# JuliaNeuralGraphics/GaussianSplatting.jl

Measured on AMD Instinct MI355X. Metric: fwd+bwd Mpixels/s @1920x1080, 1M Gaussians SH=3, higher is better.
Workload: dtype f32

## Files before the change

gaussiansplatting.jl_amd/csrc/gsr_api.cpp:

```cpp
#include "../../include/gsr.h"

#include <dlfcn.h>
#include <math.h>
#include <sched.h>
#include <time.h>
#include <hip/hip_runtime.h>

#include <algorithm>
#include <atomic>
#include <chrono>
#include <cstdarg>
#include <cstdio>
#include <cstdlib>
#include <cstring>
#include <new>
#include <vector>

#include "gsr_kernels.h"
#include "adam_math.h"

namespace {

thread_local char g_err[512] = "";

// ... 863 lines not shown

static int buffer_lookup(const gsr_handle* h, int which, const void** dev_ptr, size_t* bytes) {
    const size_t n = (size_t)h->last_n, P = (size_t)h->cfg.width * h->cfg.height, T = (size_t)h->n_tiles;
    const size_t D = (size_t)h->last_D;
    const DevBuf* b = nullptr;
    size_t sz = 0;
    switch (which) {
        case GSR_BUF_RADII:
            *dev_ptr = h->fwd_valid && n ? h->radii_cur : nullptr;
            *bytes = *dev_ptr ? n * 4 : 0;
            return GSR_OK;
        case GSR_BUF_GRAD_MEANS2D:
            *dev_ptr = h->bwd_valid && n ? h->vmean2d_cur : nullptr;
            *bytes = *dev_ptr ? n * 8 : 0;
            return GSR_OK;
        case GSR_BUF_N_CONTRIB: b = &h->n_contrib; sz = P * 4; break;
        case GSR_BUF_FINAL_T: b = &h->final_T; sz = P * 4; break;
        case GSR_BUF_TILE_RANGES: b = &h->ranges; sz = 2 * T * 4; break;
        case GSR_BUF_VALUES_SORTED: b = &h->values_sorted; sz = h->fwd_only ? 0 : D * 4; break;
        case GSR_BUF_GEOM: b = &h->geo; sz = n * 64; break;
        case GSR_BUF_NORMALS: b = &h->gnormal; sz = h->cfg.mode > 5 ? n * 16 : 0; break;
        case GSR_BUF_GRAD_ROWS: b = &h->rows; sz = (size_t)h->last_slots * 16 * GSR_ROW_F4(h->cfg.mode); break;
        case GSR_BUF_INSTANCE_AUX: b = &h->s2; sz = h->fwd_only ? 0 : D * 16; break;
        default: return fail(GSR_E_INVALID_ARG, "unknown buffer id %d", which);
    }
    if (sz > b->cap) sz = 0;
    *dev_ptr = sz ? b->p : nullptr;
    *bytes = sz;
    return GSR_OK;
}

int gsr_buffer(const gsr_handle* h, int which, const void** dev_ptr, size_t* bytes) {
    if (!h || !dev_ptr || !bytes) return fail(GSR_E_INVALID_ARG, "null argument");
    return buffer_lookup(h, which, dev_ptr, bytes);
}

int gsr_copy_buffer(const gsr_handle* h, int which, void* dst, size_t bytes, void* stream) {
    if (!h || (!dst && bytes)) return fail(GSR_E_INVALID_ARG, "null argument");
    const void* src = nullptr;
    size_t have = 0;
    int rc = buffer_lookup(h, which, &src, &have);
    if (rc) return rc;
    if (bytes > have) return fail(GSR_E_STATE, "buffer %d holds %zu bytes, %zu requested (not produced yet?)", which, have, bytes);
    if (bytes) HIPCHK(hipMemcpyAsync(dst, src, bytes, hipMemcpyDeviceToDevice, (hipStream_t)stream));
    return GSR_OK;
}

int gsr_ssim_forward(int W, int H, int CH, int B, const float* img, const float* ref, float C1, float C2, int train,
                     float* ssim_map, float* dm_dmu1, float* dm_dsigma1_sq, float* dm_dsigma12, void* stream) {
    if (W <= 0 || H <= 0 || CH <= 0 || B <= 0) return fail(GSR_E_INVALID_ARG, "bad SSIM shape");
    if (!img || !ref || !ssim_map) return fail(GSR_E_INVALID_ARG, "null SSIM array");
    if (train && (!dm_dmu1 || !dm_dsigma1_sq || !dm_dsigma12)) return fail(GSR_E_INVALID_ARG, "train needs the 3 partial maps");
    if ((size_t)CH * B > 65535) return fail(GSR_E_INVALID_ARG, "CH*B too large");
    (g_ssim_exact.load(std::memory_order_relaxed) ? gsr_launch_ssim_fwd_exact : gsr_launch_ssim_fwd_fast)((hipStream_t)stream, W, H, CH, B, img, ref, C1, C2, train,
                                                                          ssim_map, dm_dmu1, dm_dsigma1_sq, dm_dsigma12);
    HIPCHK(hipGetLastError());
    return GSR_OK;
}

int gsr_ssim_backward(int W, int H, int CH, int B, const float* img, const float* ref, const float* dL_dmap,
                      const float* dm_dmu1, const float* dm_dsigma1_sq, const float* dm_dsigma12, float* dL_dimg,
                      void* stream) {
    if (W <= 0 || H <= 0 || CH <= 0 || B <= 0) return fail(GSR_E_INVALID_ARG, "bad SSIM shape");
    if (!img || !ref || !dL_dmap || !dm_dmu1 || !dm_dsigma1_sq || !dm_dsigma12 || !dL_dimg)
        return fail(GSR_E_INVALID_ARG, "null SSIM array");
    if ((size_t)CH * B > 65535) return fail(GSR_E_INVALID_ARG, "CH*B too large");
    (g_ssim_exact.load(std::memory_order_relaxed) ? gsr_launch_ssim_bwd_exact : gsr_launch_ssim_bwd_fast)((hipStream_t)stream, W, H, CH, B, img, ref, dL_dmap, dm_dmu1,
                                                                          dm_dsigma1_sq, dm_dsigma12, dL_dimg);
    HIPCHK(hipGetLastError());
    return GSR_OK;
}

int gsr_loss_l1_ssim(gsr_handle* h, const float* image, const float* target, float lambda_dssim, float* loss_out,
                     float* vpixels, void* stream) {
    if (!h || !image || !target || !loss_out || !vpixels) return fail(GSR_E_INVALID_ARG, "null argument");
    hipStream_t s = (hipStream_t)stream;
    const int W = h->cfg.width, H = h->cfg.height, C = h->cfg.mode;
    const size_t P = (size_t)W * H;
    int rc;
    if ((rc = h->d0.ensure(3 * P * 4)) || (rc = h->d1.ensure(3 * P * 4)) || (rc = h->d2.ensure(3 * P * 4)) ||
        (rc = h->partial.ensure((size_t)h->n_tiles * 3 * 2 * 4)))
        return rc;
    const float C1 = 0.01f * 0.01f, C2 = 0.03f * 0.03f;
    const int exact = ssim_exact_of(h);
    StageScope sc9(h->prof, ST_LOSS_FWD, s);
    (exact ? gsr_launch_loss_fwd_exact : gsr_launch_loss_fwd_fast)(s, W, H, C, image, target, C1, C2, h->d0.as<float>(),
                                                                          h->d1.as<float>(), h->d2.as<float>(), h->partial.as<float>());
    sc9.close();
    StageScope sc10(h->prof, ST_LOSS_BWD, s);
    (exact ? gsr_launch_loss_bwd_exact : gsr_launch_loss_bwd_fast)(s, W, H, C, image, target, lambda_dssim, h->d0.as<float>(),
                                                                          h->d1.as<float>(), h->d2.as<float>(), h->partial.as<float>(),
                                                                          loss_out, vpixels);
    sc10.close();
    HIPCHK(hipGetLastError());
    h->loss_vpixels = vpixels;
    h->loss_generation = h->generation;
    return GSR_OK;
}

int gsr_update_stats(gsr_handle* h, int32_t* max_radii, float* accum_grad_means2d, float* denom, void* stream) {
    if (!h || !max_radii || !accum_grad_means2d || !denom) return fail(GSR_E_INVALID_ARG, "null argument");
    if (!h->fwd_valid || !h->bwd_valid) return fail(GSR_E_STATE, "gsr_update_stats needs a completed forward/backward pair");
    gsr_launch_update_stats((hipStream_t)stream, h->last_n, h->radii_cur, h->vmean2d_cur,
                            h->cfg.width, h->cfg.height, max_radii, accum_grad_means2d, denom);
    HIPCHK(hipGetLastError());
    return GSR_OK;
}

int gsr_profile_enable(gsr_handle* h, int on) {
    if (!h) return fail(GSR_E_INVALID_ARG, "null handle");
    h->prof.on = (on & 1) != 0;
    h->prof.ranges = (on & 2) != 0;
    if (!h->prof.on) h->prof.clear();
    return GSR_OK;
}

int gsr_profile_stages(gsr_handle* h, uint32_t stage_mask) {
    if (!h) return fail(GSR_E_INVALID_ARG, "null handle");
    h->prof.mask = stage_mask;
    return GSR_OK;
}

int gsr_profile_stage_count(void) { return ST_COUNT; }
const char* gsr_profile_stage_name(int stage) { return stage >= 0 && stage < ST_COUNT ? kStageNames[stage] : ""; }

int gsr_profile_read(gsr_handle* h, double* ms_sum, int* launches, int reset) {
    if (!h || !ms_sum || !launches) return fail(GSR_E_INVALID_ARG, "null argument");
    for (int i = 0; i < ST_COUNT; i++) { ms_sum[i] = 0.0; launches[i] = 0; }
    for (auto& r : h->prof.recs) {
        float ms = 0.0f;
        HIPCHK(hipEventSynchronize(r.b));
        HIPCHK(hipEventElapsedTime(&ms, r.a, r.b));
        ms_sum[r.stage] += ms;
        if (!r.extra) launches[r.stage] += 1;
    }
    if (reset) h->prof.clear();
    return GSR_OK;
// ... 476 lines not shown
```

gaussiansplatting.jl_amd/csrc/gsr_kernels.h:

```cpp
#pragma once
#include <hip/hip_runtime.h>
#include <stdint.h>

#define GSR_TILE 16
#define GSR_BATCH 256
#define GSR_SORT_LDS_CAP 8192

struct GsrCam {
    float R[9];
    float t[3];
    float focal[2];
    float principal[2];
    float center[3];
    int width, height;
    int grid_x, grid_y;
    float near_plane, far_plane;
    int radius_clip;
    float blur_eps;
    int exact_cull;
    const float* R_dev;
    const float* t_dev;
};

struct GsrGeoRec { float4 q0, q1, q2, q3; };
// ... 92 lines not shown
                              const float* final_T, GsrInst inst,
                              uint32_t split_len ,
                              bool color_only ,
                              bool accurate );
void gsr_launch_composite_bwd_listed(hipStream_t s, int channels, GsrCam cam, const uint32_t* tile_start,
                                     GsrTierLists tiers, GsrStream stream, const float* background,
                                     const float* vpixels, const uint32_t* n_contrib, const float* final_T, GsrInst inst,
                                     float* long_state );

#define GSR_ADAM_MAX_GROUPS 8
void gsr_launch_prologue_fwd(hipStream_t s, int n, int k_rest, int scale_dims, const float* sh_color,
                             const float* sh_remainder, const float* opacities, const float* scales, float* shs,
                             float* opacities_act, float* scales_act);
void gsr_launch_prologue_bwd(hipStream_t s, int n, int k_rest, int scale_dims, const float* opacities_act,
                             const float* scales_act, const float* vshs, const float* vopacities_act,
                             const float* vscales_act, float* v_sh_color, float* v_sh_remainder, float* v_opacities,
                             float* v_scales);
void gsr_launch_adam(hipStream_t s, int n_groups, float* const* theta, const float* const* grad, float* const* mu,
                     float* const* nu, const long long* count, const float* lr_t, float beta1, float beta2, float eps);

void gsr_launch_trainer_tail(hipStream_t s, int n, int k_rest, int scale_dims, const float* const* grads,
                             float* const* theta, float* const* mu, float* const* nu, const float* lr_t, float beta1,
                             float beta2, float eps, float* shs, float* opac_act, float* scales_act);
size_t gsr_findall_scratch_bytes(long long n);
void gsr_launch_findall(hipStream_t s, long long n, const uint8_t* mask, uint32_t* indices, uint32_t* count_dev,
                        uint32_t* scratch);
void gsr_launch_gather_rows(hipStream_t s, int n_groups, const void* const* src, void* const* dst, const int* row_words,
                            const uint32_t* idx, long long count);
void gsr_launch_triad(hipStream_t s, size_t n4, float* a, const float* b, const float* c, float q);

#define GSR_COMPOSE_MAX_GROUPS 24
void gsr_launch_grad_mean(hipStream_t s, long long n, const float* accum, const float* denom, float* out);
void gsr_launch_densify_mask(hipStream_t s, int kind, long long n, long long n_grad, const float* grad, const float* scales,
                             int scale_dims, const float* opacities, const int32_t* max_radii, float thr, float gamma,
                             float min_opacity, int max_screen_size, uint8_t* mask);
void gsr_launch_compose_rows(hipStream_t s, int n_groups, const void* const* src, void* const* dst, const int* row_words,
                             const int* new_zero, const uint32_t* keep_idx, long long n_keep, const uint32_t* sel_idx,
                             long long n_sel, int reps);
void gsr_launch_split_transform(hipStream_t s, long long n_new, int scale_dims, float* points, const float* rots,
                                float* scales, uint32_t seed);
void gsr_launch_reset_opacity(hipStream_t s, long long n, float* opacities);
void gsr_launch_morton_codes(hipStream_t s, long long n, const float* points, const float lo[3], const float inv_extent[3],
                             unsigned long long* codes);
void gsr_launch_nonfinite_scan(hipStream_t s, int n_groups, const float* const* src, const int* row_words, long long n_rows,
                               uint32_t* counts, uint32_t* first_bad);
void gsr_launch_ply_rows(hipStream_t s, bool pack, long long n, int kr, float* points, float* dc, float* rest, float* opac,
                         float* scales, float* rots, float* rows);

#define GSR_SSIM_DECL(SUF)                                                                                              \
    void gsr_launch_ssim_fwd_##SUF(hipStream_t s, int W, int H, int CH, int B, const float* img, const float* ref, float C1, \
                                   float C2, int train, float* ssim_map, float* d0, float* d1, float* d2);             \
    void gsr_launch_ssim_bwd_##SUF(hipStream_t s, int W, int H, int CH, int B, const float* img, const float* ref,      \
                                   const float* dL_dmap, const float* d0, const float* d1, const float* d2, float* dL_dimg); \
              \
    void gsr_launch_loss_fwd_##SUF(hipStream_t s, int W, int H, int C, const float* image, const float* target, float C1, \
                                   float C2, float* d0, float* d1, float* d2, float* partial);                         \
    void gsr_launch_loss_bwd_##SUF(hipStream_t s, int W, int H, int C, const float* image, const float* target, float lambda, \
                                   const float* d0, const float* d1, const float* d2, const float* partial, float* loss_out, \
                                   float* vpixels);
GSR_SSIM_DECL(exact)
GSR_SSIM_DECL(fast)
#undef GSR_SSIM_DECL

namespace gsr {
struct AdamHyper;
struct BilateralTv { float weight, nx, ny, nz, n12, rx, ry, rz; };
}
int gsr_bilateral_chunks(int W, int H, int gx, int gy);
size_t gsr_bilateral_partial_bytes(int W, int H, int gx, int gy, int gz);
void gsr_launch_bilateral_fwd(hipStream_t s, int W, int H, int C, const float* image, const float* grid, int gx, int gy,
                              int gz, float* out);
void gsr_launch_bilateral_bwd(hipStream_t s, int W, int H, int C, const float* image, const float* grid, int gx, int gy,
                              int gz, const float* vout, float* vimage, float* vgrid, float* partial);
void gsr_launch_bilateral_tv(hipStream_t s, int n, int gx, int gy, int gz, const float* grids, const gsr::BilateralTv& tv,
                             float* loss_out, float* grad_out, float* partial);
void gsr_launch_bilateral_adam_tail(hipStream_t s, int n, int gx, int gy, int gz, float* grids, float* mu, float* nu,
                                    const float* vgrid, int view, const gsr::BilateralTv& tv, const gsr::AdamHyper& h,
                                    float* tv_loss_out, float* partial);
```

gaussiansplatting.jl_amd/csrc/ssim.hip:

```cpp
#include "gsr_kernels.h"

#ifndef SSIM_EXACT
#define SSIM_EXACT 1
#endif
#if SSIM_EXACT
#define SSIM_NAME(x) x##_exact
#else
#define SSIM_NAME(x) x##_fast
#endif

namespace {

constexpr int HALO = 5;
constexpr int SH_DIM = GSR_TILE + 2 * HALO;
constexpr int IN_STRIDE = 48, HC_STRIDE = 16;

__constant__ float GAUSS[11] = {0.001028380123898387f, 0.0075987582094967365f, 0.036000773310661316f,
                                0.10936068743467331f,  0.21300552785396576f,   0.26601171493530273f,
                                0.21300552785396576f,  0.10936068743467331f,   0.036000773310661316f,
                                0.0075987582094967365f, 0.001028380123898387f};

struct PlanarSrc {
    const float* img;
    const float* ref;
    int W, H;
    __device__ __forceinline__ float x(int gx, int gy, int plane) const {
        return img[(size_t)gx + (size_t)W * gy + (size_t)W * H * plane];
    }
    __device__ __forceinline__ float y(int gx, int gy, int plane) const {
        return ref[(size_t)gx + (size_t)W * gy + (size_t)W * H * plane];
    }
};
struct RasterSrc {
    const float* image;
    const float* target;
    int W, H, C;
    __device__ __forceinline__ float x(int gx, int gy, int plane) const {
        return image[(size_t)C * ((size_t)gx + (size_t)W * gy) + plane];
    }
    __device__ __forceinline__ float y(int gx, int gy, int plane) const {
        return target[(size_t)gx + (size_t)W * gy + (size_t)W * H * plane];
    }
};

__device__ __forceinline__ bool ssim_tile_of_block(int W, int H, int& tx0, int& ty0) {
    const int gx = (W + GSR_TILE - 1) / GSR_TILE, gy = (H + GSR_TILE - 1) / GSR_TILE;
    const int n = gx * gy, per = (n + 7) / 8;
    const int t = (int)(blockIdx.x & 7) * per + (int)(blockIdx.x >> 3);
    if ((int)(blockIdx.x >> 3) >= per || t >= n) return false;
    tx0 = (t % gx) * GSR_TILE;
    ty0 = (t / gx) * GSR_TILE;
    return true;
}

__device__ __forceinline__ float block_sum(float v, float* red ) {
#pragma unroll
    for (int off = 32; off > 0; off >>= 1) v += __shfl_xor(v, off);
    if ((threadIdx.x & 63) == 0) red[threadIdx.x >> 6] = v;
    __syncthreads();
    float r = red[0] + red[1] + red[2] + red[3];
    __syncthreads();
    return r;
}

template <class Src, bool LOSS, int NCH>
__global__ __launch_bounds__(256) void ssim_fwd_kernel(Src src, int W, int H, float C1, float C2, int train,
                                                       float* __restrict__ ssim_map, float* __restrict__ d0,
                                                       float* __restrict__ d1, float* __restrict__ d2,
                                                       float* __restrict__ partial) {
    __shared__ float sx[SH_DIM][IN_STRIDE], sy[SH_DIM][IN_STRIDE];
    __shared__ float hc[5][SH_DIM][HC_STRIDE];
    __shared__ float red[4];
    const int tid = threadIdx.x, tx = tid & 15, ty = tid >> 4;
    int x0, y0;
    const bool live = ssim_tile_of_block(W, H, x0, y0);
    float l1 = 0.0f, sv = 0.0f;
    if (!live) {
        if (LOSS && tid == 0) { partial[2 * ((size_t)blockIdx.x + (size_t)gridDim.x * blockIdx.z)] = 0.0f; partial[2 * ((size_t)blockIdx.x + (size_t)gridDim.x * blockIdx.z) + 1] = 0.0f; }
        return;
    }
  for (int ch = 0; ch < NCH; ch++) {
    const int plane = blockIdx.z * NCH + ch;
    if (ch > 0) __syncthreads();
    for (int f = tid; f < SH_DIM * SH_DIM; f += 256) {
        const int ly = f / SH_DIM, lx = f - ly * SH_DIM;
        const int gx = x0 + lx - HALO, gy = y0 + ly - HALO;
        const bool in = gx >= 0 && gx < W && gy >= 0 && gy < H;
        sx[ly][lx] = in ? src.x(gx, gy, plane) : 0.0f;
        sy[ly][lx] = in ? src.y(gx, gy, plane) : 0.0f;
    }
    __syncthreads();
    for (int r = ty; r < SH_DIM; r += GSR_TILE) {
        const int cx = tx + HALO;
        float s0 = 0, s1 = 0, s2 = 0, s3 = 0, s4 = 0;
#pragma unroll
        for (int d = 1; d <= HALO; d++) {
            const float w = GAUSS[HALO - d];
            const float Xl = sx[r][cx - d], Yl = sy[r][cx - d], Xr = sx[r][cx + d], Yr = sy[r][cx + d];
            s0 += (Xl + Xr) * w;
            s1 += (Xl * Xl + Xr * Xr) * w;
            s2 += (Yl + Yr) * w;
            s3 += (Yl * Yl + Yr * Yr) * w;
            s4 += (Xl * Yl + Xr * Yr) * w;
        }
        const float Xc = sx[r][cx], Yc = sy[r][cx], wc = GAUSS[HALO];
        s0 += Xc * wc; s1 += Xc * Xc * wc; s2 += Yc * wc; s3 += Yc * Yc * wc; s4 += Xc * Yc * wc;
        hc[0][r][tx] = s0; hc[1][r][tx] = s1; hc[2][r][tx] = s2; hc[3][r][tx] = s3; hc[4][r][tx] = s4;
    }
    __syncthreads();
    const int px = x0 + tx, py = y0 + ty;
    const bool in = px < W && py < H;
    float o[5];
    {
        const int cy = ty + HALO;
#pragma unroll
        for (int k = 0; k < 5; k++) {
            float a = 0;
#pragma unroll
            for (int d = 1; d <= HALO; d++) a += (hc[k][cy - d][tx] + hc[k][cy + d][tx]) * GAUSS[HALO - d];
            a += hc[k][cy][tx] * GAUSS[HALO];
            o[k] = a;
        }
    }
    if (in) {
        const float mu1 = o[0], mu2 = o[2];
        const float mu1_sq = mu1 * mu1, mu2_sq = mu2 * mu2;
        const float sigma1_sq = o[1] - mu1_sq, sigma2_sq = o[3] - mu2_sq, sigma12 = o[4] - mu1 * mu2;
        const float A = mu1_sq + mu2_sq + C1, Bv = sigma1_sq + sigma2_sq + C2;
        const float Cv = 2.0f * mu1 * mu2 + C1, Dv = 2.0f * sigma12 + C2;
        const size_t oi = (size_t)px + (size_t)W * py + (size_t)W * H * plane;
#if SSIM_EXACT
        const float val = (Cv * Dv) / (A * Bv);
        if (!LOSS) ssim_map[oi] = val;
        if (train) {
            d0[oi] = ((mu2 * 2.0f * Dv) / (A * Bv) - (mu2 * 2.0f * Cv) / (A * Bv) -
                      (mu1 * 2.0f * Cv * Dv) / (A * A * Bv) + (mu1 * 2.0f * Cv * Dv) / (A * Bv * Bv));
            d1[oi] = (-Cv * Dv) / (A * Bv * Bv);
            d2[oi] = (2.0f * Cv) / (A * Bv);
        }
#else
        const float rA = __builtin_amdgcn_rcpf(A), rB = __builtin_amdgcn_rcpf(Bv), rAB = rA * rB;
        const float val = (Cv * Dv) * rAB;
        if (!LOSS) ssim_map[oi] = val;
        if (train) {
            d0[oi] = 2.0f * (mu2 * (Dv - Cv) * rAB + mu1 * val * (rB - rA));
            d1[oi] = -val * rB;
            d2[oi] = 2.0f * Cv * rAB;
        }
#endif
        if (LOSS) {
            sv += val;
            l1 += fabsf(sx[ty + HALO][tx + HALO] - sy[ty + HALO][tx + HALO]);
        }
    }
  }
    if (LOSS) {
        const float a = block_sum(l1, red), b = block_sum(sv, red);
        if (tid == 0) {
            const size_t blk = (size_t)blockIdx.x + (size_t)gridDim.x * blockIdx.z;
            partial[2 * blk] = a;
            partial[2 * blk + 1] = b;
        }
    }
}

__device__ __forceinline__ void loss_finish_body(const float* __restrict__ partial, int n_blocks, float lambda,
                                                 float inv_count, float* __restrict__ loss_out) {
    __shared__ float red[2][4];
    float a = 0.0f, b = 0.0f;
    for (int i = threadIdx.x; i < n_blocks; i += 256) {
        const float2 p = reinterpret_cast<const float2*>(partial)[i];
        a += p.x; b += p.y;
    }
#pragma unroll
    for (int off = 32; off > 0; off >>= 1) { a += __shfl_xor(a, off); b += __shfl_xor(b, off); }
    if ((threadIdx.x & 63) == 0) { red[0][threadIdx.x >> 6] = a; red[1][threadIdx.x >> 6] = b; }
    __syncthreads();
    if (threadIdx.x == 0) {
        a = 0.0f; b = 0.0f;
        for (int w = 0; w < 4; w++) { a += red[0][w]; b += red[1][w]; }
        const float l1 = a * inv_count;
        const float s = 1.0f - b * inv_count;
        loss_out[0] = (1.0f - lambda) * l1 + lambda * s;
    }
}

template <class Src, bool LOSS, int NCH>
__global__ __launch_bounds__(256) void ssim_bwd_kernel(Src src, int W, int H, const float* __restrict__ dL_dmap,
                                                       float chain_const, float l1_scale,
                                                       const float* __restrict__ d0, const float* __restrict__ d1,
                                                       const float* __restrict__ d2, float* __restrict__ out,
                                                       int outC, const float* __restrict__ partial, int n_partial,
                                                       float lambda, float inv_count, float* __restrict__ loss_out) {
    __shared__ float sd[3][SH_DIM][IN_STRIDE];
    __shared__ float hc[3][SH_DIM][HC_STRIDE];
    const int tid = threadIdx.x, tx = tid & 15, ty = tid >> 4;
    if (LOSS && blockIdx.x == gridDim.x - 1) {
        loss_finish_body(partial, n_partial, lambda, inv_count, loss_out);
        return;
    }
    int x0, y0;
    if (!ssim_tile_of_block(W, H, x0, y0)) return;
    const size_t P = (size_t)W * H;
    float gout[NCH];
  for (int ch = 0; ch < NCH; ch++) {
    const int plane = blockIdx.z * NCH + ch;
    gout[ch] = 0.0f;
    if (ch > 0) __syncthreads();
    for (int f = tid; f < SH_DIM * SH_DIM; f += 256) {
        const int ly = f / SH_DIM, lx = f - ly * SH_DIM;
        const int gx = x0 + lx - HALO, gy = y0 + ly - HALO;
        const bool in = gx >= 0 && gx < W && gy >= 0 && gy < H;
        const size_t gi = (size_t)gx + (size_t)W * gy + P * plane;
        const float chain = in ? (LOSS ? chain_const : dL_dmap[gi]) : 0.0f;
        sd[0][ly][lx] = (in ? d0[gi] : 0.0f) * chain;
        sd[1][ly][lx] = (in ? d1[gi] : 0.0f) * chain;
        sd[2][ly][lx] = (in ? d2[gi] : 0.0f) * chain;
    }
    __syncthreads();
    for (int r = ty; r < SH_DIM; r += GSR_TILE) {
        const int cx = tx + HALO;
#pragma unroll
        for (int k = 0; k < 3; k++) {
            float a = 0;
#pragma unroll
            for (int d = 1; d <= HALO; d++) a += (sd[k][r][cx - d] + sd[k][r][cx + d]) * GAUSS[HALO - d];
            a += sd[k][r][cx] * GAUSS[HALO];
            hc[k][r][tx] = a;
        }
    }
    __syncthreads();
    const int px = x0 + tx, py = y0 + ty;
    if (px < W && py < H) {
        const int cy = ty + HALO;
        float s[3];
#pragma unroll
        for (int k = 0; k < 3; k++) {
            float a = 0;
#pragma unroll
            for (int d = 1; d <= HALO; d++) a += (hc[k][cy - d][tx] + hc[k][cy + d][tx]) * GAUSS[HALO - d];
            a += hc[k][cy][tx] * GAUSS[HALO];
            s[k] = a;
        }
        const float p1 = src.x(px, py, plane), p2 = src.y(px, py, plane);
        float g = s[0] + 2.0f * p1 * s[1] + p2 * s[2];
        if (LOSS) {
            const float df = p1 - p2;
            g = g + l1_scale * (df > 0.0f ? 1.0f : (df < 0.0f ? -1.0f : 0.0f));
            gout[ch] = g;
        } else {
            out[(size_t)px + (size_t)W * py + P * plane] = g;
        }
    }
  }
    if (LOSS) {
        const int px = x0 + tx, py = y0 + ty;
        if (px < W && py < H) {
            float* o = out + (size_t)outC * ((size_t)px + (size_t)W * py) + (size_t)blockIdx.z * NCH;
#pragma unroll
            for (int ch = 0; ch < NCH; ch++) o[ch] = gout[ch];
            for (int c = NCH; c < outC; c++) o[c] = 0.0f;
        }
    }
}

}

static dim3 ssim_grid(int W, int H, int planes) {
    const int n = ((W + GSR_TILE - 1) / GSR_TILE) * ((H + GSR_TILE - 1) / GSR_TILE);
    return dim3(8 * ((n + 7) / 8), 1, planes);
}

void SSIM_NAME(gsr_launch_ssim_fwd)(hipStream_t s, int W, int H, int CH, int B, const float* img, const float* ref, float C1,
                         float C2, int train, float* ssim_map, float* d0, float* d1, float* d2) {
    PlanarSrc src{img, ref, W, H};
    hipLaunchKernelGGL((ssim_fwd_kernel<PlanarSrc, false, 1>), ssim_grid(W, H, CH * B), dim3(256), 0, s, src, W, H, C1,
                       C2, train, ssim_map, d0, d1, d2, (float*)nullptr);
}

void SSIM_NAME(gsr_launch_ssim_bwd)(hipStream_t s, int W, int H, int CH, int B, const float* img, const float* ref,
                         const float* dL_dmap, const float* d0, const float* d1, const float* d2, float* dL_dimg) {
    PlanarSrc src{img, ref, W, H};
    hipLaunchKernelGGL((ssim_bwd_kernel<PlanarSrc, false, 1>), ssim_grid(W, H, CH * B), dim3(256), 0, s, src, W, H,
                       dL_dmap, 0.0f, 0.0f, d0, d1, d2, dL_dimg, 0, (const float*)nullptr, 0, 0.0f, 0.0f, (float*)nullptr);
}

void SSIM_NAME(gsr_launch_loss_fwd)(hipStream_t s, int W, int H, int C, const float* image, const float* target, float C1,
                         float C2, float* d0, float* d1, float* d2, float* partial) {
    RasterSrc src{image, target, W, H, C};
    hipLaunchKernelGGL((ssim_fwd_kernel<RasterSrc, true, 3>), ssim_grid(W, H, 1), dim3(256), 0, s, src, W, H, C1, C2, 1,
                       (float*)nullptr, d0, d1, d2, partial);
}

void SSIM_NAME(gsr_launch_loss_bwd)(hipStream_t s, int W, int H, int C, const float* image, const float* target, float lambda,
                         const float* d0, const float* d1, const float* d2, const float* partial, float* loss_out,
                         float* vpixels) {
    RasterSrc src{image, target, W, H, C};
    const float count = 3.0f * (float)W * (float)H;
    const float inv_count = 1.0f / count;
    dim3 g = ssim_grid(W, H, 1);
    const int n_partial = (int)(g.x * g.y * g.z);
    g.x += 1;
    hipLaunchKernelGGL((ssim_bwd_kernel<RasterSrc, true, 3>), g, dim3(256), 0, s, src, W, H,
                       (const float*)nullptr, -lambda * inv_count, (1.0f - lambda) * inv_count, d0, d1, d2, vpixels,
                       C, partial, n_partial, lambda, inv_count, loss_out);
}
```

Measured before the change: 1465.

## Rewrite SSIM kernels as per-wave vertical strips with register ring buffers

```diff
diff --git a/gaussiansplatting.jl_amd/csrc/gsr_api.cpp b/gaussiansplatting.jl_amd/csrc/gsr_api.cpp
--- a/gaussiansplatting.jl_amd/csrc/gsr_api.cpp
+++ b/gaussiansplatting.jl_amd/csrc/gsr_api.cpp
@@ -939,6 +939,7 @@
     if (!img || !ref || !ssim_map) return fail(GSR_E_INVALID_ARG, "null SSIM array");
     if (train && (!dm_dmu1 || !dm_dsigma1_sq || !dm_dsigma12)) return fail(GSR_E_INVALID_ARG, "train needs the 3 partial maps");
     if ((size_t)CH * B > 65535) return fail(GSR_E_INVALID_ARG, "CH*B too large");
+    if ((size_t)W * H > 0xFFFFFFFFull) return fail(GSR_E_INVALID_ARG, "SSIM plane too large");
     (g_ssim_exact.load(std::memory_order_relaxed) ? gsr_launch_ssim_fwd_exact : gsr_launch_ssim_fwd_fast)((hipStream_t)stream, W, H, CH, B, img, ref, C1, C2, train,
                                                                           ssim_map, dm_dmu1, dm_dsigma1_sq, dm_dsigma12);
     HIPCHK(hipGetLastError());
@@ -952,6 +953,7 @@
     if (!img || !ref || !dL_dmap || !dm_dmu1 || !dm_dsigma1_sq || !dm_dsigma12 || !dL_dimg)
         return fail(GSR_E_INVALID_ARG, "null SSIM array");
     if ((size_t)CH * B > 65535) return fail(GSR_E_INVALID_ARG, "CH*B too large");
+    if ((size_t)W * H > 0xFFFFFFFFull) return fail(GSR_E_INVALID_ARG, "SSIM plane too large");
     (g_ssim_exact.load(std::memory_order_relaxed) ? gsr_launch_ssim_bwd_exact : gsr_launch_ssim_bwd_fast)((hipStream_t)stream, W, H, CH, B, img, ref, dL_dmap, dm_dmu1,
                                                                           dm_dsigma1_sq, dm_dsigma12, dL_dimg);
     HIPCHK(hipGetLastError());
@@ -964,12 +966,13 @@
     hipStream_t s = (hipStream_t)stream;
     const int W = h->cfg.width, H = h->cfg.height, C = h->cfg.mode;
     const size_t P = (size_t)W * H;
+    if (P * C > 0xFFFFFFFFull) return fail(GSR_E_INVALID_ARG, "image too large for the loss head");
+    const int exact = ssim_exact_of(h);
     int rc;
     if ((rc = h->d0.ensure(3 * P * 4)) || (rc = h->d1.ensure(3 * P * 4)) || (rc = h->d2.ensure(3 * P * 4)) ||
-        (rc = h->partial.ensure((size_t)h->n_tiles * 3 * 2 * 4)))
+        (rc = h->partial.ensure((exact ? gsr_loss_partial_pairs_exact : gsr_loss_partial_pairs_fast)(W, H) * 2 * 4)))
         return rc;
     const float C1 = 0.01f * 0.01f, C2 = 0.03f * 0.03f;
-    const int exact = ssim_exact_of(h);
     StageScope sc9(h->prof, ST_LOSS_FWD, s);
     (exact ? gsr_launch_loss_fwd_exact : gsr_launch_loss_fwd_fast)(s, W, H, C, image, target, C1, C2, h->d0.as<float>(),
                                                                           h->d1.as<float>(), h->d2.as<float>(), h->partial.as<float>());
diff --git a/gaussiansplatting.jl_amd/csrc/gsr_kernels.h b/gaussiansplatting.jl_amd/csrc/gsr_kernels.h
--- a/gaussiansplatting.jl_amd/csrc/gsr_kernels.h
+++ b/gaussiansplatting.jl_amd/csrc/gsr_kernels.h
@@ -168,7 +168,8 @@
                                    float C2, int train, float* ssim_map, float* d0, float* d1, float* d2);             \
     void gsr_launch_ssim_bwd_##SUF(hipStream_t s, int W, int H, int CH, int B, const float* img, const float* ref,      \
                                    const float* dL_dmap, const float* d0, const float* d1, const float* d2, float* dL_dimg); \
-              \
+     \
+    size_t gsr_loss_partial_pairs_##SUF(int W, int H);                                                                 \
     void gsr_launch_loss_fwd_##SUF(hipStream_t s, int W, int H, int C, const float* image, const float* target, float C1, \
                                    float C2, float* d0, float* d1, float* d2, float* partial);                         \
     void gsr_launch_loss_bwd_##SUF(hipStream_t s, int W, int H, int C, const float* image, const float* target, float lambda, \
diff --git a/gaussiansplatting.jl_amd/csrc/ssim.hip b/gaussiansplatting.jl_amd/csrc/ssim.hip
--- a/gaussiansplatting.jl_amd/csrc/ssim.hip
+++ b/gaussiansplatting.jl_amd/csrc/ssim.hip
@@ -12,284 +12,379 @@
 namespace {
 
 constexpr int HALO = 5;
-constexpr int SH_DIM = GSR_TILE + 2 * HALO;
-constexpr int IN_STRIDE = 48, HC_STRIDE = 16;
+constexpr int STRIP_W = 64 - 2 * HALO;
+constexpr int AHEAD = 3;
+constexpr int MIN_WAVES = 4;
+constexpr int RING = 2 * HALO + 1;
+constexpr int LOSS_STRIPS = 1;
+constexpr int ROW_LDS = 64 + 2 * HALO;
 
 __constant__ float GAUSS[11] = {0.001028380123898387f, 0.0075987582094967365f, 0.036000773310661316f,
                                 0.10936068743467331f,  0.21300552785396576f,   0.26601171493530273f,
                                 0.21300552785396576f,  0.10936068743467331f,   0.036000773310661316f,
                                 0.0075987582094967365f, 0.001028380123898387f};
 
+typedef float v2f __attribute__((ext_vector_type(2)));
+
 struct PlanarSrc {
     const float* img;
     const float* ref;
     int W, H;
-    __device__ __forceinline__ float x(int gx, int gy, int plane) const {
-        return img[(size_t)gx + (size_t)W * gy + (size_t)W * H * plane];
-    }
-    __device__ __forceinline__ float y(int gx, int gy, int plane) const {
-        return ref[(size_t)gx + (size_t)W * gy + (size_t)W * H * plane];
-    }
+    __device__ __forceinline__ const float* xplane(int plane) const { return img + (size_t)W * H * plane; }
+    __device__ __forceinline__ const float* yplane(int plane) const { return ref + (size_t)W * H * plane; }
+    __device__ __forceinline__ unsigned xrow(int gy) const { return (unsigned)W * (unsigned)gy; }
+    __device__ __forceinline__ unsigned xlane(int gx) const { return 4u * (unsigned)gx; }
 };
 struct RasterSrc {
     const float* image;
     const float* target;
     int W, H, C;
-    __device__ __forceinline__ float x(int gx, int gy, int plane) const {
-        return image[(size_t)C * ((size_t)gx + (size_t)W * gy) + plane];
-    }
-    __device__ __forceinline__ float y(int gx, int gy, int plane) const {
-        return target[(size_t)gx + (size_t)W * gy + (size_t)W * H * plane];
-    }
+    __device__ __forceinline__ const float* xplane(int plane) const { return image + plane; }
+    __device__ __forceinline__ const float* yplane(int plane) const { return target + (size_t)W * H * plane; }
+    __device__ __forceinline__ unsigned xrow(int gy) const { return (unsigned)(C * W) * (unsigned)gy; }
+    __device__ __forceinline__ unsigned xlane(int gx) const { return 4u * (unsigned)(C * gx); }
 };
 
-__device__ __forceinline__ bool ssim_tile_of_block(int W, int H, int& tx0, int& ty0) {
-    const int gx = (W + GSR_TILE - 1) / GSR_TILE, gy = (H + GSR_TILE - 1) / GSR_TILE;
-    const int n = gx * gy, per = (n + 7) / 8;
-    const int t = (int)(blockIdx.x & 7) * per + (int)(blockIdx.x >> 3);
-    if ((int)(blockIdx.x >> 3) >= per || t >= n) return false;
-    tx0 = (t % gx) * GSR_TILE;
-    ty0 = (t / gx) * GSR_TILE;
+template <class T>
+__device__ __forceinline__ T& at(T* plane, unsigned row, unsigned lane_off) {
+    return *(T*)((char*)(plane + row) + lane_off);
+}
+template <class T>
+__device__ __forceinline__ const T& at(const T* plane, unsigned row, unsigned lane_off) {
+    return *(const T*)((const char*)(plane + row) + lane_off);
+}
+
+struct Strip {
+    int x0, y0, rows;
+};
+template <int NPL, int SPB>
+__device__ __forceinline__ bool strip_of_wave(int W, int H, int strip_h, int wv, Strip& st) {
+    const int nsx = (W + STRIP_W - 1) / STRIP_W, nsy = (H + strip_h - 1) / strip_h;
+    const int n = nsx * nsy, groups = (n + SPB - 1) / SPB, per = (groups + 7) / 8;
+    const int g = (int)(blockIdx.x & 7) * per + (int)(blockIdx.x >> 3);
+    const int s = g * SPB + wv / NPL;
+    if ((int)(blockIdx.x >> 3) >= per || g >= groups || s >= n) return false;
+    st.x0 = (s % nsx) * STRIP_W;
+    st.y0 = (s / nsx) * strip_h;
+    st.rows = min(strip_h, H - st.y0);
     return true;
 }
 
-__device__ __forceinline__ float block_sum(float v, float* red ) {
+__device__ __forceinline__ void wave_sync() {
+    __builtin_amdgcn_fence(__ATOMIC_RELEASE, "wavefront");
+    __builtin_amdgcn_wave_barrier();
+    __builtin_amdgcn_fence(__ATOMIC_ACQUIRE, "wavefront");
+}
+
+__device__ __forceinline__ float wave_sum(float v) {
 #pragma unroll
     for (int off = 32; off > 0; off >>= 1) v += __shfl_xor(v, off);
-    if ((threadIdx.x & 63) == 0) red[threadIdx.x >> 6] = v;
-    __syncthreads();
-    float r = red[0] + red[1] + red[2] + red[3];
-    __syncthreads();
-    return r;
-}
-
-template <class Src, bool LOSS, int NCH>
-__global__ __launch_bounds__(256) void ssim_fwd_kernel(Src src, int W, int H, float C1, float C2, int train,
-                                                       float* __restrict__ ssim_map, float* __restrict__ d0,
-                                                       float* __restrict__ d1, float* __restrict__ d2,
-                                                       float* __restrict__ partial) {
-    __shared__ float sx[SH_DIM][IN_STRIDE], sy[SH_DIM][IN_STRIDE];
-    __shared__ float hc[5][SH_DIM][HC_STRIDE];
-    __shared__ float red[4];
-    const int tid = threadIdx.x, tx = tid & 15, ty = tid >> 4;
-    int x0, y0;
-    const bool live = ssim_tile_of_block(W, H, x0, y0);
+    return v;
+}
+
+__device__ __forceinline__ float sum_of_products(float a, float b, float c, float d) {
+#if SSIM_EXACT
+    return a * b + c * d;
+#else
+    return __builtin_fmaf(a, b, c * d);
+#endif
+}
+
+template <class T>
+__device__ __forceinline__ T ring_vertical(const T (&h)[RING], int j) {
+    T a = 0;
+#pragma unroll
+    for (int d = 1; d <= HALO; d++) a += (h[(j + HALO + 1 + RING - d) % RING] + h[(j + HALO + 1 + d) % RING]) * GAUSS[HALO - d];
+    a += h[(j + HALO + 1) % RING] * GAUSS[HALO];
+    return a;
+}
+
+template <class Src, bool LOSS, int NPL, int SPB>
+__global__ __launch_bounds__(64 * NPL * SPB, MIN_WAVES) void ssim_fwd_kernel(Src src, int W, int H, int strip_h, float C1, float C2, int train,
+                                                                 float* __restrict__ ssim_map, float* __restrict__ d0,
+                                                                 float* __restrict__ d1, float* __restrict__ d2,
+                                                                 float* __restrict__ partial) {
+    constexpr int NW = NPL * SPB;
+    __shared__ v2f rowbuf[NW][ROW_LDS];
+    const int lane = threadIdx.x & 63, wv = __builtin_amdgcn_readfirstlane(threadIdx.x >> 6);
+    Strip st;
+    if (!strip_of_wave<NPL, SPB>(W, H, strip_h, wv, st)) {
+        if (LOSS && lane == 0) { partial[2 * ((size_t)blockIdx.x * NW + wv)] = 0.0f; partial[2 * ((size_t)blockIdx.x * NW + wv) + 1] = 0.0f; }
+        return;
+    }
+    const int plane = blockIdx.z * NPL + wv % NPL;
+    v2f* buf = rowbuf[wv];
+    if (lane < HALO) { buf[lane] = v2f{0.0f, 0.0f}; buf[64 + HALO + lane] = v2f{0.0f, 0.0f}; }
+    const int gx = st.x0 - HALO + lane, cx = lane + HALO;
+    const bool col_in = gx >= 0 && gx < W;
+    const bool own = lane >= HALO && lane < 64 - HALO && gx < W;
+    const int nrows = st.rows + 2 * HALO;
+    const int gxc = min(max(gx, 0), W - 1);
+    const unsigned xo = src.xlane(gxc), yo = 4u * (unsigned)gxc;
+    const float* xp = src.xplane(plane);
+    const float* yp = src.yplane(plane);
+    const size_t po = (size_t)W * H * plane;
+    auto fetch = [&](int rr) {
+        const int gyc = min(max(st.y0 - HALO + rr, 0), H - 1);
+        return v2f{at(xp, src.xrow(gyc), xo), at(yp, (unsigned)W * (unsigned)gyc, yo)};
+    };
+    v2f nxt[AHEAD];
+#pragma unroll
+    for (int i = 0; i < AHEAD; i++) nxt[i] = fetch(i);
+    v2f hm[RING], hq[RING];
+    float hc[RING];
     float l1 = 0.0f, sv = 0.0f;
-    if (!live) {
-        if (LOSS && tid == 0) { partial[2 * ((size_t)blockIdx.x + (size_t)gridDim.x * blockIdx.z)] = 0.0f; partial[2 * ((size_t)blockIdx.x + (size_t)gridDim.x * blockIdx.z) + 1] = 0.0f; }
-        return;
-    }
-  for (int ch = 0; ch < NCH; ch++) {
-    const int plane = blockIdx.z * NCH + ch;
-    if (ch > 0) __syncthreads();
-    for (int f = tid; f < SH_DIM * SH_DIM; f += 256) {
-        const int ly = f / SH_DIM, lx = f - ly * SH_DIM;
-        const int gx = x0 + lx - HALO, gy = y0 + ly - HALO;
-        const bool in = gx >= 0 && gx < W && gy >= 0 && gy < H;
-        sx[ly][lx] = in ? src.x(gx, gy, plane) : 0.0f;
-        sy[ly][lx] = in ? src.y(gx, gy, plane) : 0.0f;
-    }
-    __syncthreads();
-    for (int r = ty; r < SH_DIM; r += GSR_TILE) {
-        const int cx = tx + HALO;
-        float s0 = 0, s1 = 0, s2 = 0, s3 = 0, s4 = 0;
-#pragma unroll
-        for (int d = 1; d <= HALO; d++) {
-            const float w = GAUSS[HALO - d];
-            const float Xl = sx[r][cx - d], Yl = sy[r][cx - d], Xr = sx[r][cx + d], Yr = sy[r][cx + d];
-            s0 += (Xl + Xr) * w;
-            s1 += (Xl * Xl + Xr * Xr) * w;
-            s2 += (Yl + Yr) * w;
-            s3 += (Yl * Yl + Yr * Yr) * w;
-            s4 += (Xl * Yl + Xr * Yr) * w;
+    for (int base = 0; base < nrows; base += RING) {
+#pragma unroll
+        for (int j = 0; j < RING; j++) {
+            const int rr = base + j;
+            if (rr < nrows) {
+                const int gy = st.y0 - HALO + rr;
+                const v2f XY = col_in && gy >= 0 && gy < H ? nxt[0] : v2f{0.0f, 0.0f};
+#pragma unroll
+                for (int i = 0; i + 1 < AHEAD; i++) nxt[i] = nxt[i + 1];
+                nxt[AHEAD - 1] = fetch(rr + AHEAD);
+                buf[cx] = XY;
+                wave_sync();
+                v2f m = 0, q = 0;
+                float c = 0;
+#pragma unroll
+                for (int d = 1; d <= HALO; d++) {
+                    const float w = GAUSS[HALO - d];
+                    const v2f L = buf[cx - d], R = buf[cx + d];
+                    m += (L + R) * w;
+                    q += (L * L + R * R) * w;
+                    c += sum_of_products(L.x, L.y, R.x, R.y) * w;
+                }
+                wave_sync();
+                const float wc = GAUSS[HALO];
+                m += XY * wc; q += XY * XY * wc; c += XY.x * XY.y * wc;
+                hm[j] = m; hq[j] = q; hc[j] = c;
+                if (LOSS && own && rr >= HALO && rr < nrows - HALO) l1 += fabsf(XY.x - XY.y);
+                if (rr >= 2 * HALO) {
+                    const v2f om = ring_vertical(hm, j), oq = ring_vertical(hq, j);
+                    const float o[5] = {om.x, oq.x, om.y, oq.y, ring_vertical(hc, j)};
+                    if (own) {
+                        const int py = st.y0 + rr - 2 * HALO;
+                        const float mu1 = o[0], mu2 = o[2];
+                        const float mu1_sq = mu1 * mu1, mu2_sq = mu2 * mu2;
+                        const float sigma1_sq = o[1] - mu1_sq, sigma2_sq = o[3] - mu2_sq, sigma12 = o[4] - mu1 * mu2;
+                        const float A = mu1_sq + mu2_sq + C1, Bv = sigma1_sq + sigma2_sq + C2;
+                        const float Cv = 2.0f * mu1 * mu2 + C1, Dv = 2.0f * sigma12 + C2;
+                        const unsigned orow = (unsigned)W * (unsigned)py;
+#if SSIM_EXACT
+                        const float val = (Cv * Dv) / (A * Bv);
+                        if (!LOSS) at(ssim_map + po, orow, yo) = val;
+                        if (train) {
+                            at(d0 + po, orow, yo) = ((mu2 * 2.0f * Dv) / (A * Bv) - (mu2 * 2.0f * Cv) / (A * Bv) -
+                                      (mu1 * 2.0f * Cv * Dv) / (A * A * Bv) + (mu1 * 2.0f * Cv * Dv) / (A * Bv * Bv));
+                            at(d1 + po, orow, yo) = (-Cv * Dv) / (A * Bv * Bv);
+                            at(d2 + po, orow, yo) = (2.0f * Cv) / (A * Bv);
+                        }
+#else
+                        const float rA = __builtin_amdgcn_rcpf(A), rB = __builtin_amdgcn_rcpf(Bv), rAB = rA * rB;
+                        const float val = (Cv * Dv) * rAB;
+                        if (!LOSS) at(ssim_map + po, orow, yo) = val;
+                        if (train) {
+                            at(d0 + po, orow, yo) = 2.0f * (mu2 * (Dv - Cv) * rAB + mu1 * val * (rB - rA));
+                            at(d1 + po, orow, yo) = -val * rB;
+                            at(d2 + po, orow, yo) = 2.0f * Cv * rAB;
+                        }
+#endif
+                        if (LOSS) sv += val;
+                    }
+                }
+            }
         }
-        const float Xc = sx[r][cx], Yc = sy[r][cx], wc = GAUSS[HALO];
-        s0 += Xc * wc; s1 += Xc * Xc * wc; s2 += Yc * wc; s3 += Yc * Yc * wc; s4 += Xc * Yc * wc;
-        hc[0][r][tx] = s0; hc[1][r][tx] = s1; hc[2][r][tx] = s2; hc[3][r][tx] = s3; hc[4][r][tx] = s4;
-    }
-    __syncthreads();
-    const int px = x0 + tx, py = y0 + ty;
-    const bool in = px < W && py < H;
-    float o[5];
-    {
-        const int cy = ty + HALO;
-#pragma unroll
-        for (int k = 0; k < 5; k++) {
-            float a = 0;
-#pragma unroll
-            for (int d = 1; d <= HALO; d++) a += (hc[k][cy - d][tx] + hc[k][cy + d][tx]) * GAUSS[HALO - d];
-            a += hc[k][cy][tx] * GAUSS[HALO];
-            o[k] = a;
+    }
+    if (LOSS) {
+        const float a = wave_sum(l1), b = wave_sum(sv);
+        if (lane == 0) {
+            const size_t pair = (size_t)blockIdx.x * NW + wv;
+            partial[2 * pair] = a;
+            partial[2 * pair + 1] = b;
         }
     }
-    if (in) {
-        const float mu1 = o[0], mu2 = o[2];
-        const float mu1_sq = mu1 * mu1, mu2_sq = mu2 * mu2;
-        const float sigma1_sq = o[1] - mu1_sq, sigma2_sq = o[3] - mu2_sq, sigma12 = o[4] - mu1 * mu2;
-        const float A = mu1_sq + mu2_sq + C1, Bv = sigma1_sq + sigma2_sq + C2;
-        const float Cv = 2.0f * mu1 * mu2 + C1, Dv = 2.0f * sigma12 + C2;
-        const size_t oi = (size_t)px + (size_t)W * py + (size_t)W * H * plane;
-#if SSIM_EXACT
-        const float val = (Cv * Dv) / (A * Bv);
-        if (!LOSS) ssim_map[oi] = val;
-        if (train) {
-            d0[oi] = ((mu2 * 2.0f * Dv) / (A * Bv) - (mu2 * 2.0f * Cv) / (A * Bv) -
-                      (mu1 * 2.0f * Cv * Dv) / (A * A * Bv) + (mu1 * 2.0f * Cv * Dv) / (A * Bv * Bv));
-            d1[oi] = (-Cv * Dv) / (A * Bv * Bv);
-            d2[oi] = (2.0f * Cv) / (A * Bv);
-        }
-#else
-        const float rA = __builtin_amdgcn_rcpf(A), rB = __builtin_amdgcn_rcpf(Bv), rAB = rA * rB;
-        const float val = (Cv * Dv) * rAB;
-        if (!LOSS) ssim_map[oi] = val;
-        if (train) {
-            d0[oi] = 2.0f * (mu2 * (Dv - Cv) * rAB + mu1 * val * (rB - rA));
-            d1[oi] = -val * rB;
-            d2[oi] = 2.0f * Cv * rAB;
-        }
-#endif
-        if (LOSS) {
-            sv += val;
-            l1 += fabsf(sx[ty + HALO][tx + HALO] - sy[ty + HALO][tx + HALO]);
-        }
-    }
-  }
-    if (LOSS) {
-        const float a = block_sum(l1, red), b = block_sum(sv, red);
-        if (tid == 0) {
-            const size_t blk = (size_t)blockIdx.x + (size_t)gridDim.x * blockIdx.z;
-            partial[2 * blk] = a;
-            partial[2 * blk + 1] = b;
-        }
-    }
-}
-
-__device__ __forceinline__ void loss_finish_body(const float* __restrict__ partial, int n_blocks, float lambda,
+}
+
+template <int NT>
+__device__ __forceinline__ void loss_finish_body(const float* __restrict__ partial, int n_pairs, float lambda,
                                                  float inv_count, float* __restrict__ loss_out) {
-    __shared__ float red[2][4];
+    __shared__ float red[2][NT / 64];
     float a = 0.0f, b = 0.0f;
-    for (int i = threadIdx.x; i < n_blocks; i += 256) {
+    for (int i = threadIdx.x; i < n_pairs; i += NT) {
         const float2 p = reinterpret_cast<const float2*>(partial)[i];
         a += p.x; b += p.y;
     }
-#pragma unroll
-    for (int off = 32; off > 0; off >>= 1) { a += __shfl_xor(a, off); b += __shfl_xor(b, off); }
+    a = wave_sum(a); b = wave_sum(b);
     if ((threadIdx.x & 63) == 0) { red[0][threadIdx.x >> 6] = a; red[1][threadIdx.x >> 6] = b; }
     __syncthreads();
     if (threadIdx.x == 0) {
         a = 0.0f; b = 0.0f;
-        for (int w = 0; w < 4; w++) { a += red[0][w]; b += red[1][w]; }
+        for (int w = 0; w < NT / 64; w++) { a += red[0][w]; b += red[1][w]; }
         const float l1 = a * inv_count;
         const float s = 1.0f - b * inv_count;
         loss_out[0] = (1.0f - lambda) * l1 + lambda * s;
     }
 }
 
-template <class Src, bool LOSS, int NCH>
-__global__ __launch_bounds__(256) void ssim_bwd_kernel(Src src, int W, int H, const float* __restrict__ dL_dmap,
-                                                       float chain_const, float l1_scale,
-                                                       const float* __restrict__ d0, const float* __restrict__ d1,
-                                                       const float* __restrict__ d2, float* __restrict__ out,
-                                                       int outC, const float* __restrict__ partial, int n_partial,
-                                                       float lambda, float inv_count, float* __restrict__ loss_out) {
-    __shared__ float sd[3][SH_DIM][IN_STRIDE];
-    __shared__ float hc[3][SH_DIM][HC_STRIDE];
-    const int tid = threadIdx.x, tx = tid & 15, ty = tid >> 4;
+template <class Src, bool LOSS, int NPL, int SPB>
+__global__ __launch_bounds__(64 * NPL * SPB, MIN_WAVES) void ssim_bwd_kernel(Src src, int W, int H, int strip_h, const float* __restrict__ dL_dmap,
+                                                                 float chain_const, float l1_scale,
+                                                                 const float* __restrict__ d0, const float* __restrict__ d1,
+                                                                 const float* __restrict__ d2, float* __restrict__ out,
+                                                                 int outC, const float* __restrict__ partial, int n_partial,
+                                                                 float lambda, float inv_count, float* __restrict__ loss_out) {
+    constexpr int NW = NPL * SPB;
+    __shared__ v2f rowbuf01[NW][ROW_LDS];
+    __shared__ float rowbuf2[NW][ROW_LDS];
     if (LOSS && blockIdx.x == gridDim.x - 1) {
-        loss_finish_body(partial, n_partial, lambda, inv_count, loss_out);
+        loss_finish_body<64 * NW>(partial, n_partial, lambda, inv_count, loss_out);
         return;
     }
-    int x0, y0;
-    if (!ssim_tile_of_block(W, H, x0, y0)) return;
+    const int lane = threadIdx.x & 63, wv = __builtin_amdgcn_readfirstlane(threadIdx.x >> 6);
+    Strip st;
+    if (!strip_of_wave<NPL, SPB>(W, H, strip_h, wv, st)) return;
+    const int ch = wv % NPL, plane = blockIdx.z * NPL + ch;
     const size_t P = (size_t)W * H;
-    float gout[NCH];
-  for (int ch = 0; ch < NCH; ch++) {
-    const int plane = blockIdx.z * NCH + ch;
-    gout[ch] = 0.0f;
-    if (ch > 0) __syncthreads();
-    for (int f = tid; f < SH_DIM * SH_DIM; f += 256) {
-        const int ly = f / SH_DIM, lx = f - ly * SH_DIM;
-        const int gx = x0 + lx - HALO, gy = y0 + ly - HALO;
-        const bool in = gx >= 0 && gx < W && gy >= 0 && gy < H;
-        const size_t gi = (size_t)gx + (size_t)W * gy + P * plane;
-        const float chain = in ? (LOSS ? chain_const : dL_dmap[gi]) : 0.0f;
-        sd[0][ly][lx] = (in ? d0[gi] : 0.0f) * chain;
-        sd[1][ly][lx] = (in ? d1[gi] : 0.0f) * chain;
-        sd[2][ly][lx] = (in ? d2[gi] : 0.0f) * chain;
-    }
-    __syncthreads();
-    for (int r = ty; r < SH_DIM; r += GSR_TILE) {
-        const int cx = tx + HALO;
-#pragma unroll
-        for (int k = 0; k < 3; k++) {
-            float a = 0;
-#pragma unroll
-            for (int d = 1; d <= HALO; d++) a += (sd[k][r][cx - d] + sd[k][r][cx + d]) * GAUSS[HALO - d];
-            a += sd[k][r][cx] * GAUSS[HALO];
-            hc[k][r][tx] = a;
+    v2f* b01 = rowbuf01[wv];
+    float* b2 = rowbuf2[wv];
+    if (lane < HALO) {
+        b01[lane] = v2f{0.0f, 0.0f}; b2[lane] = 0.0f;
+        b01[64 + HALO + lane] = v2f{0.0f, 0.0f}; b2[64 + HALO + lane] = 0.0f;
+    }
+    const int gx = st.x0 - HALO + lane, cx = lane + HALO;
+    const bool col_in = gx >= 0 && gx < W;
+    const bool own = lane >= HALO && lane < 64 - HALO && gx < W;
+    const int nrows = st.rows + 2 * HALO;
+    const int gxc = min(max(gx, 0), W - 1);
+    const unsigned xo = src.xlane(gxc), yo = 4u * (unsigned)gxc;
+    const float* xp = src.xplane(plane);
+    const float* yp = src.yplane(plane);
+    const size_t po = P * plane;
+    struct Row { v2f a01; float a2, chain, p1, p2; };
+    auto fetch = [&](int rr) {
+        const int gy = st.y0 - HALO + rr;
+        const int gyc = min(max(gy, 0), H - 1), gyo = min(max(gy - HALO, 0), H - 1);
+        const unsigned ro = (unsigned)W * (unsigned)gyc;
+        Row r;
+        r.a01 = v2f{at(d0 + po, ro, yo), at(d1 + po, ro, yo)};
+        r.a2 = at(d2 + po, ro, yo);
+        r.chain = LOSS ? chain_const : at(dL_dmap + po, ro, yo);
+        r.p1 = at(xp, src.xrow(gyo), xo);
+        r.p2 = at(yp, (unsigned)W * (unsigned)gyo, yo);
+        return r;
+    };
+    Row nr[AHEAD];
+#pragma unroll
+    for (int i = 0; i < AHEAD; i++) nr[i] = fetch(i);
+    v2f h01[RING];
+    float h2[RING];
+    for (int base = 0; base < nrows; base += RING) {
+#pragma unroll
+        for (int j = 0; j < RING; j++) {
+            const int rr = base + j;
+            if (rr < nrows) {
+                const int gy = st.y0 - HALO + rr;
+                const bool in = col_in && gy >= 0 && gy < H;
+                Row r = nr[0];
+                r.chain = in ? r.chain : 0.0f;
+                r.a01 = (in ? r.a01 : v2f{0.0f, 0.0f}) * r.chain;
+                r.a2 = (in ? r.a2 : 0.0f) * r.chain;
+#pragma unroll
+                for (int i = 0; i + 1 < AHEAD; i++) nr[i] = nr[i + 1];
+                nr[AHEAD - 1] = fetch(rr + AHEAD);
+                b01[cx] = r.a01; b2[cx] = r.a2;
+                wave_sync();
+                v2f s01 = 0;
+                float s2 = 0;
+#pragma unroll
+                for (int d = 1; d <= HALO; d++) {
+                    const float w = GAUSS[HALO - d];
+                    s01 += (b01[cx - d] + b01[cx + d]) * w;
+                    s2 += (b2[cx - d] + b2[cx + d]) * w;
+                }
+                wave_sync();
+                h01[j] = s01 + r.a01 * GAUSS[HALO];
+                h2[j] = s2 + r.a2 * GAUSS[HALO];
+                if (rr >= 2 * HALO) {
+                    const v2f v01 = ring_vertical(h01, j);
+                    const float s[3] = {v01.x, v01.y, ring_vertical(h2, j)};
+                    if (own) {
+                        const int py = st.y0 + rr - 2 * HALO;
+                        const float p1 = r.p1, p2 = r.p2;
+                        float g = s[0] + 2.0f * p1 * s[1] + p2 * s[2];
+                        if (LOSS) {
+                            const float df = p1 - p2;
+                            g = g + l1_scale * (df > 0.0f ? 1.0f : (df < 0.0f ? -1.0f : 0.0f));
+                            float* o = &at(out + ch, (unsigned)(outC * W) * (unsigned)py, 4u * (unsigned)(outC * gxc));
+                            o[0] = g;
+                            if (ch == NPL - 1)
+                                for (int c = 1; c <= outC - NPL; c++) o[c] = 0.0f;
+                        } else {
+                            at(out + po, (unsigned)W * (unsigned)py, yo) = g;
+                        }
+                    }
+                }
+            }
         }
     }
-    __syncthreads();
-    const int px = x0 + tx, py = y0 + ty;
-    if (px < W && py < H) {
-        const int cy = ty + HALO;
-        float s[3];
-#pragma unroll
-        for (int k = 0; k < 3; k++) {
-            float a = 0;
-#pragma unroll
-            for (int d = 1; d <= HALO; d++) a += (hc[k][cy - d][tx] + hc[k][cy + d][tx]) * GAUSS[HALO - d];
-            a += hc[k][cy][tx] * GAUSS[HALO];
-            s[k] = a;
-        }
-        const float p1 = src.x(px, py, plane), p2 = src.y(px, py, plane);
-        float g = s[0] + 2.0f * p1 * s[1] + p2 * s[2];
-        if (LOSS) {
-            const float df = p1 - p2;
-            g = g + l1_scale * (df > 0.0f ? 1.0f : (df < 0.0f ? -1.0f : 0.0f));
-            gout[ch] = g;
-        } else {
-            out[(size_t)px + (size_t)W * py + P * plane] = g;
-        }
-    }
-  }
-    if (LOSS) {
-        const int px = x0 + tx, py = y0 + ty;
-        if (px < W && py < H) {
-            float* o = out + (size_t)outC * ((size_t)px + (size_t)W * py) + (size_t)blockIdx.z * NCH;
-#pragma unroll
-            for (int ch = 0; ch < NCH; ch++) o[ch] = gout[ch];
-            for (int c = NCH; c < outC; c++) o[c] = 0.0f;
-        }
-    }
-}
-
-}
-
-static dim3 ssim_grid(int W, int H, int planes) {
-    const int n = ((W + GSR_TILE - 1) / GSR_TILE) * ((H + GSR_TILE - 1) / GSR_TILE);
-    return dim3(8 * ((n + 7) / 8), 1, planes);
+}
+
+}
+
+static int ssim_strip_h(int W, int H, int planes) {
+    static const int n_simd = [] {
+        int dev = 0, cus = 0;
+        if (hipGetDevice(&dev) != hipSuccess || hipDeviceGetAttribute(&cus, hipDeviceAttributeMultiprocessorCount, dev) != hipSuccess || cus <= 0)
+            cus = 256;
+        return 4 * cus;
+    }();
+    const long cols = (long)((W + STRIP_W - 1) / STRIP_W) * planes;
+    int best = 8;
+    long best_cost = -1;
+    for (int h = 8; h <= 64; h++) {
+        const long waves = cols * ((H + h - 1) / h);
+        const long per_simd = (waves + n_simd - 1) / n_simd;
+        const long cost = (per_simd < 3 ? 3 : per_simd) * (h + 4);
+        if (best_cost < 0 || cost < best_cost) { best_cost = cost; best = h; }
+    }
+    return best;
+}
+
+template <int SPB>
+static dim3 ssim_grid(int W, int H, int strip_h, int planes) {
+    const int n = ((W + STRIP_W - 1) / STRIP_W) * ((H + strip_h - 1) / strip_h);
+    const int groups = (n + SPB - 1) / SPB;
+    return dim3(8 * ((groups + 7) / 8), 1, planes);
+}
+
+size_t SSIM_NAME(gsr_loss_partial_pairs)(int W, int H) {
+    return (size_t)ssim_grid<LOSS_STRIPS>(W, H, ssim_strip_h(W, H, 3), 1).x * 3 * LOSS_STRIPS;
 }
 
 void SSIM_NAME(gsr_launch_ssim_fwd)(hipStream_t s, int W, int H, int CH, int B, const float* img, const float* ref, float C1,
                          float C2, int train, float* ssim_map, float* d0, float* d1, float* d2) {
     PlanarSrc src{img, ref, W, H};
-    hipLaunchKernelGGL((ssim_fwd_kernel<PlanarSrc, false, 1>), ssim_grid(W, H, CH * B), dim3(256), 0, s, src, W, H, C1,
-                       C2, train, ssim_map, d0, d1, d2, (float*)nullptr);
+    const int sh = ssim_strip_h(W, H, CH * B);
+    hipLaunchKernelGGL((ssim_fwd_kernel<PlanarSrc, false, 1, 4>), ssim_grid<4>(W, H, sh, CH * B), dim3(256), 0, s, src, W, H, sh,
+                       C1, C2, train, ssim_map, d0, d1, d2, (float*)nullptr);
 }
 
 void SSIM_NAME(gsr_launch_ssim_bwd)(hipStream_t s, int W, int H, int CH, int B, const float* img, const float* ref,
                          const float* dL_dmap, const float* d0, const float* d1, const float* d2, float* dL_dimg) {
     PlanarSrc src{img, ref, W, H};
-    hipLaunchKernelGGL((ssim_bwd_kernel<PlanarSrc, false, 1>), ssim_grid(W, H, CH * B), dim3(256), 0, s, src, W, H,
+    const int sh = ssim_strip_h(W, H, CH * B);
+    hipLaunchKernelGGL((ssim_bwd_kernel<PlanarSrc, false, 1, 4>), ssim_grid<4>(W, H, sh, CH * B), dim3(256), 0, s, src, W, H, sh,
                        dL_dmap, 0.0f, 0.0f, d0, d1, d2, dL_dimg, 0, (const float*)nullptr, 0, 0.0f, 0.0f, (float*)nullptr);
 }
 
 void SSIM_NAME(gsr_launch_loss_fwd)(hipStream_t s, int W, int H, int C, const float* image, const float* target, float C1,
                          float C2, float* d0, float* d1, float* d2, float* partial) {
     RasterSrc src{image, target, W, H, C};
-    hipLaunchKernelGGL((ssim_fwd_kernel<RasterSrc, true, 3>), ssim_grid(W, H, 1), dim3(256), 0, s, src, W, H, C1, C2, 1,
-                       (float*)nullptr, d0, d1, d2, partial);
+    const int sh = ssim_strip_h(W, H, 3);
+    hipLaunchKernelGGL((ssim_fwd_kernel<RasterSrc, true, 3, LOSS_STRIPS>), ssim_grid<LOSS_STRIPS>(W, H, sh, 1),
+                       dim3(64 * 3 * LOSS_STRIPS), 0, s, src, W, H, sh, C1, C2, 1, (float*)nullptr, d0, d1, d2, partial);
 }
 
 void SSIM_NAME(gsr_launch_loss_bwd)(hipStream_t s, int W, int H, int C, const float* image, const float* target, float lambda,
@@ -298,10 +393,11 @@
     RasterSrc src{image, target, W, H, C};
     const float count = 3.0f * (float)W * (float)H;
     const float inv_count = 1.0f / count;
-    dim3 g = ssim_grid(W, H, 1);
-    const int n_partial = (int)(g.x * g.y * g.z);
+    const int sh = ssim_strip_h(W, H, 3);
+    dim3 g = ssim_grid<LOSS_STRIPS>(W, H, sh, 1);
+    const int n_partial = (int)(g.x * 3 * LOSS_STRIPS);
     g.x += 1;
-    hipLaunchKernelGGL((ssim_bwd_kernel<RasterSrc, true, 3>), g, dim3(256), 0, s, src, W, H,
+    hipLaunchKernelGGL((ssim_bwd_kernel<RasterSrc, true, 3, LOSS_STRIPS>), g, dim3(64 * 3 * LOSS_STRIPS), 0, s, src, W, H, sh,
                        (const float*)nullptr, -lambda * inv_count, (1.0f - lambda) * inv_count, d0, d1, d2, vpixels,
                        C, partial, n_partial, lambda, inv_count, loss_out);
 }
```

Measured after the change: 1501, median of 6. 2.4% higher.
